# mobiusml/hqq

Hardware: NVIDIA H100
Metric: llama3_8b_4bit_gs64_decode_tokens_per_s (higher is better)
Workload: dtype f16

## Files before the change

hqq_b200/_lib.py:

```python
from __future__ import annotations

import ctypes
import os
from ctypes import c_char_p, c_float, c_int, c_int32, c_int64, c_size_t, c_void_p

import torch

_PKG_DIR = os.path.dirname(os.path.abspath(__file__))
LIB_PATH = os.path.join(_PKG_DIR, "libhqq_b200.so")

HQQ_F32, HQQ_F16, HQQ_BF16, HQQ_U8, HQQ_I32, HQQ_I64 = range(6)
HQQ_OK, HQQ_E_INVALID, HQQ_E_UNSUPPORTED, HQQ_E_WORKSPACE, HQQ_E_CUDA = 0, -1, -2, -3, -4

DTYPE_CODE = {
    torch.float32: HQQ_F32, torch.float16: HQQ_F16, torch.bfloat16: HQQ_BF16,
    torch.uint8: HQQ_U8, torch.int32: HQQ_I32, torch.int64: HQQ_I64,
}

SIGNATURES = {
    "hqq_b200_abi_version": (c_int, []),
    "hqq_b200_last_error": (c_char_p, []),
    "hqq_b200_pack": (c_int, [c_int, c_void_p, c_int, c_void_p, c_int64, c_int64, c_void_p]),
    "hqq_b200_unpack": (c_int, [c_int, c_void_p, c_void_p, c_int, c_int64, c_int64, c_void_p]),
    "hqq_b200_dequantize": (c_int, [c_void_p, c_void_p, c_void_p, c_void_p, c_int64, c_int64, c_int, c_int, c_int, c_int, c_void_p]),
    "hqq_b200_quantize_workspace_bytes": (c_size_t, [c_int64, c_int64, c_int, c_int, c_int, c_int]),
    "hqq_b200_quantize_shard_begin": (c_int, [c_void_p, c_int, c_int64, c_int64, c_int, c_int, c_int, c_int, c_float, c_float, c_int, c_void_p,
                                              c_void_p, c_size_t, c_void_p]),
    "hqq_b200_quantize_shard_finish": (c_int, [c_void_p, c_int, c_int64, c_int64, c_int, c_int, c_int, c_int, c_float, c_float, c_int, c_void_p,
                                               c_int64, c_void_p, c_void_p, c_void_p, c_void_p, c_void_p, c_void_p, c_size_t, c_void_p]),
    "hqq_b200_quantize": (c_int, [c_void_p, c_int, c_int64, c_int64, c_int, c_int, c_int, c_int, c_int, c_float, c_float, c_int,
                                  c_void_p, c_void_p, c_void_p, c_void_p, c_void_p, c_void_p, c_size_t, c_void_p]),
    "hqq_b200_quantize_ex": (c_int, [c_void_p, c_int, c_int64, c_int64, c_int, c_int, c_int, c_int, c_int, c_int, c_float, c_float,
                                     c_int, c_void_p, c_void_p, c_void_p, c_void_p, c_void_p, c_void_p, c_void_p, c_void_p,
                                     c_size_t, c_void_p]),
    "hqq_b200_linear_fwd_workspace_bytes": (c_size_t, [c_int64, c_int64, c_int64, c_int, c_int, c_int, c_int]),
    "hqq_b200_dense_gemm": (c_int, [c_void_p, c_void_p, c_void_p, c_void_p, c_int64, c_int64, c_int64, c_int, c_void_p]),
    "hqq_b200_lm_logprob_workspace_bytes": (c_size_t, [c_int64, c_int64]),
    "hqq_b200_lm_logprob": (c_int, [c_void_p, c_void_p, c_void_p, c_void_p, c_void_p, c_void_p, c_int64, c_int64, c_int64, c_int64, c_int, c_void_p]),
    "hqq_b200_linear_fwd": (c_int, [c_void_p, c_void_p, c_void_p, c_void_p, c_void_p, c_void_p, c_int64, c_int64, c_int64,
                                    c_int, c_int, c_int, c_int, c_void_p, c_size_t, c_void_p]),
    "hqq_b200_linear_fwd_multi": (c_int, [c_void_p, c_int, c_void_p, c_void_p, c_void_p, c_void_p, c_void_p, c_void_p, c_int64, c_int64,
                                          c_int, c_int, c_int, c_int, c_void_p, c_size_t, c_void_p]),
    "hqq_b200_linear_fwd_route": (c_int, [c_int64, c_int64, c_int64, c_int, c_int, c_int, c_int]),
    "hqq_b200_decode_linear_fwd": (c_int, [c_void_p, c_int, c_void_p, c_void_p, c_void_p, c_float, c_int, c_void_p, c_void_p, c_void_p, c_void_p,
                                           c_void_p, c_void_p, c_int64, c_int, c_int, c_int, c_void_p]),
    "hqq_b200_decode_linear_fwd_desc": (c_int, [c_void_p, c_void_p]),
    "hqq_b200_glue_add_rmsnorm_tp": (c_int, [c_void_p, c_void_p, c_void_p, c_int, c_int, c_int, c_void_p, c_void_p, c_int, c_float, c_int, c_void_p]),
    "hqq_b200_glue_add_rmsnorm": (c_int, [c_void_p, c_void_p, c_void_p, c_void_p, c_int, c_float, c_int, c_void_p]),
    "hqq_b200_glue_add_rmsnorm_rows": (c_int, [c_void_p, c_void_p, c_void_p, c_void_p, c_int, c_int, c_float, c_int, c_void_p]),
    "hqq_b200_glue_silu_mul": (c_int, [c_void_p, c_void_p, c_void_p, c_int, c_int, c_void_p]),
    "hqq_b200_glue_rope_attn_decode_batch": (c_int, [c_void_p, c_void_p, c_void_p, c_void_p, c_void_p, c_void_p, c_void_p, c_void_p, c_void_p,
                                                     c_int, c_int, c_int, c_int, c_int, c_int, c_void_p]),
    "hqq_b200_glue_rope_attn_decode": (c_int, [c_void_p, c_void_p, c_void_p, c_void_p, c_void_p, c_void_p, c_void_p, c_void_p, c_void_p,
                                               c_int, c_int, c_int, c_int, c_int, c_void_p]),
    "hqq_b200_glue_rope_attn_decode_split": (c_int, [c_void_p, c_void_p, c_void_p, c_void_p, c_void_p, c_void_p, c_void_p, c_void_p, c_void_p,
                                                     c_void_p, c_int, c_int, c_int, c_int, c_int, c_int, c_void_p]),
    "hqq_b200_glue_rope_attn_decode_split_workspace_bytes": (c_size_t, [c_int, c_int, c_int, c_int]),
    "hqq_b200_glue_rope_append_rows": (c_int, [c_void_p, c_void_p, c_void_p, c_void_p, c_void_p, c_void_p, c_void_p, c_void_p, c_int, c_int, c_int,
                                               c_int, c_int, c_int, c_int, c_int, c_void_p]),
    "hqq_b200_glue_rope_attn_decode_split_kv8": (c_int, [c_void_p] * 14 + [c_int] * 7 + [c_void_p]),
    "hqq_b200_glue_rope_append_rows_kv8": (c_int, [c_void_p] * 14 + [c_int] * 9 + [c_void_p]),
    "hqq_b200_glue_attn_prefill": (c_int, [c_void_p, c_void_p, c_void_p, c_void_p, c_int, c_int, c_int, c_int, c_int, c_int, c_int, c_int, c_void_p]),
    "hqq_b200_glue_rope_attn_decode_batch_seqpos": (c_int, [c_void_p] * 9 + [c_int] * 6 + [c_void_p]),
    "hqq_b200_glue_rope_attn_decode_split_seqpos": (c_int, [c_void_p] * 10 + [c_int] * 6 + [c_void_p]),
    "hqq_b200_glue_rope_attn_decode_split_kv8_seqpos": (c_int, [c_void_p] * 14 + [c_int] * 7 + [c_void_p]),
    "hqq_b200_glue_rope_append_rows_varlen": (c_int, [c_void_p] * 10 + [c_int] * 6 + [c_void_p]),
    "hqq_b200_glue_rope_append_rows_kv8_varlen": (c_int, [c_void_p] * 16 + [c_int] * 7 + [c_void_p]),
    "hqq_b200_glue_attn_prefill_varlen": (c_int, [c_void_p] * 6 + [c_int] * 6 + [c_void_p]),
    "hqq_b200_glue_rope_attn_decode_batch_paged": (c_int, [c_void_p] * 10 + [c_int] * 7 + [c_void_p]),
    "hqq_b200_glue_rope_attn_decode_split_paged": (c_int, [c_void_p] * 11 + [c_int] * 7 + [c_void_p]),
    "hqq_b200_glue_rope_attn_decode_split_kv8_paged": (c_int, [c_void_p] * 15 + [c_int] * 8 + [c_void_p]),
    "hqq_b200_glue_rope_append_rows_paged": (c_int, [c_void_p] * 11 + [c_int] * 7 + [c_void_p]),
    "hqq_b200_glue_rope_append_rows_kv8_paged": (c_int, [c_void_p] * 17 + [c_int] * 8 + [c_void_p]),
    "hqq_b200_glue_kv8_stage_paged": (c_int, [c_void_p] * 11 + [c_int] * 7 + [c_void_p]),
    "hqq_b200_glue_attn_prefill_paged": (c_int, [c_void_p] * 7 + [c_int] * 7 + [c_void_p]),
    "hqq_b200_glue_rope_append_rows_devpos": (c_int, [c_void_p] * 9 + [c_int] * 7 + [c_void_p]),
    "hqq_b200_glue_rope_append_rows_devpos_paged": (c_int, [c_void_p] * 10 + [c_int] * 8 + [c_void_p]),
    "hqq_b200_glue_attn_verify_split_workspace_bytes": (c_size_t, [c_int] * 5),
    "hqq_b200_glue_rope_append_rows_kv8_devpos": (c_int, [c_void_p] * 13 + [c_int] * 8 + [c_void_p]),
# ... 95 lines not shown
```

hqq_b200/csrc/linear.cu:

```cuda
#include "linear_internal.cuh"

namespace hqq {
bool small_route_ok(int64_t M, int64_t N, int64_t K, int gs, int nbits, int axis, int dtype);
size_t small_workspace_bytes(int64_t M);
int linear_small_multi(const void* x, int nprob, const void* const* Wq, const void* const* scale, const void* const* zero,
                       const void* const* bias, void* const* y, const int64_t* N, int64_t M, int64_t K, int gs, int nbits, int dtype,
                       void* ws, size_t ws_bytes, cudaStream_t st, int xop = 0, const void* x2 = nullptr, const void* xw = nullptr,
                       void* h_out = nullptr, float eps = 0.0f, const TpExchange* tpx = nullptr);
bool small_xop_ok(int64_t M, int64_t K);
bool gemm_route_ok(int64_t M, int64_t N, int64_t K, int gs, int nbits, int axis, int dtype);
size_t gemm_workspace_bytes(int64_t M, int64_t N, int64_t K, int gs, int nbits, int dtype);
int linear_gemm(const void* x, const void* Wq, const void* scale, const void* zero, const void* bias, void* y, int64_t M,
                int64_t N, int64_t K, int gs, int nbits, int dtype, void* ws, size_t ws_bytes, cudaStream_t st);
bool dense_route_ok(int64_t M, int64_t N, int64_t K, int dtype);
int linear_dense(const void* x, const void* W, const void* bias, void* y, int64_t M, int64_t N, int64_t K, int dtype, cudaStream_t st);
size_t lm_logprob_ws_bytes(int64_t M, int64_t N);
int lm_logprob(const void* x, const void* W, const int64_t* targets, float* lse, float* tgt, void* ws, int64_t M, int64_t N, int64_t K,
               int64_t index_offset, int dtype, cudaStream_t st);
}

using namespace hqq;

static bool dequant_ok(int64_t N, int64_t K, int gs, int nbits, int axis) {
  if (!valid_nbits(nbits) || !(axis == 0 || axis == 1) || gs <= 0 || N <= 0 || K <= 0 || (N * K) % gs != 0) return false;
  const int64_t R = axis == 1 ? N * K / gs : gs;
  return nbits == 3 || R % fields_of(nbits) == 0;
}

static size_t dense_ws_bytes(int64_t N, int64_t K, int dtype) { return (size_t)((N * K * (int64_t)dtype_size(dtype) + 255) & ~(int64_t)255); }

static bool prefer_small(int64_t M, int64_t N, int64_t K) {
  HQQ_ENV_KNOB(m, ([] { const char* e = getenv("HQQ_B200_SMALL_M_MAX"); return e ? atoi(e) : 0; })());
  if (m > 0) return M <= m;
  return M <= 16 || N * K <= (int64_t(1) << 24);
}

extern "C" int hqq_b200_linear_fwd_route(int64_t M, int64_t N, int64_t K, int group_size, int nbits, int axis, int dtype) {
  const bool small = small_route_ok(M, N, K, group_size, nbits, axis, dtype);
  if (small && (prefer_small(M, N, K) || !gemm_route_ok(M, N, K, group_size, nbits, axis, dtype))) return 1;
  if (gemm_route_ok(M, N, K, group_size, nbits, axis, dtype)) return 2;
  if (dequant_ok(N, K, group_size, nbits, axis) && dense_route_ok(M, N, K, dtype)) return 3;
  return 0;
// ... 58 lines not shown
  int rc = check_common(x, M, K, group_size, nbits, axis);
  if (rc) return rc;
  HQQ_REQUIRE(count >= 1 && count <= 4 && W_q && scale && zero && y && N, HQQ_E_INVALID, "hqq_b200_linear_fwd_multi: 1..4 matrices, non-null arrays");
  for (int i = 0; i < count; ++i) {
    if (!small_route_ok(M, N[i], K, group_size, nbits, axis, dtype)) {
      set_error("hqq_b200_linear_fwd_multi: matrix %d (N=%lld K=%lld gs=%d nbits=%d axis=%d dtype=%d M=%lld) is outside the fused small-M kernel",
                i, (long long)N[i], (long long)K, group_size, nbits, axis, dtype, (long long)M);
      return HQQ_E_UNSUPPORTED;
    }
  }
  return linear_small_multi(x, count, W_q, scale, zero, bias, y, N, M, K, group_size, nbits, dtype, workspace, workspace_bytes, (cudaStream_t)stream);
}

extern "C" int hqq_b200_decode_linear_fwd(const void* x, int x_op, const void* x2, const void* x_weight, void* h_out, float eps, int count,
                                          const void* const* W_q, const void* const* scale, const void* const* zero,
                                          const void* const* bias, void* const* y, const int64_t* N, int64_t K, int group_size, int nbits,
                                          int dtype, void* stream) {
  int rc = check_common(x, 1, K, group_size, nbits, 1);
  if (rc) return rc;
  HQQ_REQUIRE(count >= 1 && count <= 4 && W_q && scale && zero && y && N, HQQ_E_INVALID, "hqq_b200_decode_linear_fwd: 1..4 matrices, non-null arrays");
  HQQ_REQUIRE(x_op >= 0 && (x_op & 15) <= 2 && (x_op >> 4) <= 1, HQQ_E_INVALID,
              "hqq_b200_decode_linear_fwd: x_op must be 0 (none), 1 (add+rmsnorm) or 2 (silu*mul), optionally | HQQ_YOP_SILU_MUL_PAIR");
  for (int i = 0; i < count; ++i) {
    if (!small_route_ok(1, N[i], K, group_size, nbits, 1, dtype) || (x_op != 0 && !small_xop_ok(1, K))) {
      set_error("hqq_b200_decode_linear_fwd: matrix %d (N=%lld K=%lld gs=%d nbits=%d dtype=%d) is outside the fused M=1 kernel", i, (long long)N[i],
                (long long)K, group_size, nbits, dtype);
      return HQQ_E_UNSUPPORTED;
    }
  }
  return linear_small_multi(x, count, W_q, scale, zero, bias, y, N, 1, K, group_size, nbits, dtype, nullptr, 0, (cudaStream_t)stream, x_op, x2,
                            x_weight, h_out, eps);
}

extern "C" int hqq_b200_decode_linear_fwd_desc(const hqq_b200_decode_desc* d, void* stream) {
  HQQ_REQUIRE(d != nullptr, HQQ_E_INVALID, "hqq_b200_decode_linear_fwd_desc: null descriptor");
  int rc = check_common(d->x ? d->x : d->x_tagged, 1, d->K, d->group_size, d->nbits, 1);
  if (rc) return rc;
  HQQ_REQUIRE(d->count >= 1 && d->count <= 4 && d->W_q && d->scale && d->zero && d->y && d->N, HQQ_E_INVALID,
              "hqq_b200_decode_linear_fwd_desc: 1..4 matrices, non-null arrays");
  HQQ_REQUIRE(d->x_op >= 0 && (d->x_op & 15) <= 2 && (d->x_op >> 4) <= 1, HQQ_E_INVALID,
              "hqq_b200_decode_linear_fwd_desc: x_op must be 0, 1 or 2, optionally | HQQ_YOP_SILU_MUL_PAIR");
  HQQ_REQUIRE(d->x || ((d->x_op & 15) == 2 && d->x_tagged), HQQ_E_INVALID, "hqq_b200_decode_linear_fwd_desc: no activation given");
  for (int i = 0; i < d->count; ++i) {
    if (!small_route_ok(1, d->N[i], d->K, d->group_size, d->nbits, 1, d->dtype) || !small_xop_ok(1, d->K)) {
      set_error("hqq_b200_decode_linear_fwd_desc: matrix %d (N=%lld K=%lld gs=%d nbits=%d dtype=%d) is outside the fused M=1 kernel", i,
                (long long)d->N[i], (long long)d->K, d->group_size, d->nbits, d->dtype);
      return HQQ_E_UNSUPPORTED;
    }
  }
  TpExchange t{d->tp, d->rank, d->peer_data, d->red_data, d->y_tagged, d->x_tagged, d->x2_tagged, d->step_ctr, d->x_index, d->x_per_step};
  const bool exchange = d->step_ctr != nullptr;
  const void* x = d->x ? d->x : d->x_tagged;
  return linear_small_multi(x, d->count, d->W_q, d->scale, d->zero, d->bias, d->y, d->N, 1, d->K, d->group_size, d->nbits, d->dtype, nullptr, 0,
                            (cudaStream_t)stream, d->x_op, d->x2, d->x_weight, d->h_out, d->eps, exchange ? &t : nullptr);
}
```

hqq_b200/csrc/linear_small.cu:

```cuda
#include <string.h>
#include <type_traits>

#include "linear_internal.cuh"

namespace hqq {


constexpr int kMaxProb = 4;

struct SKProb {
  const uint8_t* Wq;
  const void* scale;
  const void* zero;
  const void* bias;
  void* y;
  uint32_t* ytag;
  int N;
  int step;
  int tile0;
};

struct SKArgs {
  SKProb p[kMaxProb];
  int nprob;
// ... 407 lines not shown
#pragma unroll
      for (int mt = 0; mt < MT; ++mt) {
        float4 acc = make_float4(0.f, 0.f, 0.f, 0.f);
#pragma unroll
        for (int w = 0; w < 8; ++w) {
          const float4 v = *reinterpret_cast<const float4*>(buf + (w * MT + mt) * 128 + lane * 4);
          acc.x += v.x; acc.y += v.y; acc.z += v.z; acc.w += v.w;
        }
        const int m0 = mt * 8 + 2 * c;
        if (m0 < a.M) {
          if (ok_a) MM::st(t.y, (long long)m0 * t.N + n_a, acc.x, t.bias, n_a);
          if (ok_b) MM::st(t.y, (long long)m0 * t.N + n_b, acc.z, t.bias, n_b);
        }
        if (m0 + 1 < a.M) {
          if (ok_a) MM::st(t.y, (long long)(m0 + 1) * t.N + n_a, acc.y, t.bias, n_a);
          if (ok_b) MM::st(t.y, (long long)(m0 + 1) * t.N + n_b, acc.w, t.bias, n_b);
        }
      }
    }
  }
  cp_async_wait<0>();
}

template <typename T, int NBITS, int GS, int ST, int MR = 0>
struct D1Cfg {
  static constexpr int F = 8 / NBITS, P = 16 / F, MPG = GS / 16, GPB = 256 / GS;
  static constexpr int NWV = (F == 1) ? 8 : 4;
  static constexpr int W_BYTES = ST * NWV * 256 * 16;
  static constexpr int M_BYTES = (MR & 1) ? ST * 8 * 4 * 8 * 16 : 0;
  static constexpr int P_BYTES = 2 * 8 * 16 * 4;
  static int smem(int K) { return W_BYTES + M_BYTES + P_BYTES + K * 2 + (K / GS) * 4; }
};

template <typename T, int NBITS, int GS, int ST, int MC, int MR = 0>
__global__ void __launch_bounds__(256, MC) linear_decode1_kernel(const __grid_constant__ SKArgs a) {
  using C = D1Cfg<T, NBITS, GS, ST, MR>;
  constexpr int F = C::F, P = C::P, MPG = C::MPG, GPB = C::GPB, NWV = C::NWV;
  using MM = MT16<T>;
  extern __shared__ __align__(16) uint8_t smem[];
  uint4* wring = reinterpret_cast<uint4*>(smem);
  uint4* mring = reinterpret_cast<uint4*>(smem + C::W_BYTES);
  float* part_s = reinterpret_cast<float*>(smem + C::W_BYTES + C::M_BYTES);
  T* xs = reinterpret_cast<T*>(smem + C::W_BYTES + C::M_BYTES + C::P_BYTES);
  float* xsum = reinterpret_cast<float*>(smem + C::W_BYTES + C::M_BYTES + C::P_BYTES + a.K * 2);

  const int tid = threadIdx.x, warp = tid >> 5, lane = tid & 31;
  const int r = lane >> 2, c = lane & 3;
  const int p = (F == 1) ? r : (r % P);
  const int fa = (F == 1) ? 0 : (r / P), fb = (F == 1) ? 0 : (F / 2 + r / P);
  Lanes<T, NBITS> lanes;
  lanes.init(8 - NBITS * (fa + 1), 8 - NBITS * (fb + 1));

  const int kb0 = a.KB * warp / 8, kb1 = a.KB * (warp + 1) / 8;
  const int upt = kb1 - kb0;
  const int n_tiles = (a.total_tiles - (int)blockIdx.x + (int)gridDim.x - 1) / (int)gridDim.x;
  if (n_tiles <= 0) return;

  struct Tile { const uint8_t* Wq; const T* scale; const T* zero; const T* bias; T* y; uint32_t* ytag; int N, step, tile0; };
  auto pick = [&](int pi, Tile& t) {
    const uint8_t* Wq = a.p[0].Wq; const void* sc = a.p[0].scale; const void* ze = a.p[0].zero; const void* bi = a.p[0].bias;
    void* y = a.p[0].y; uint32_t* yt = a.p[0].ytag; int N = a.p[0].N, step = a.p[0].step, tile0 = a.p[0].tile0;
#pragma unroll
    for (int i = 1; i < kMaxProb; ++i)
      if (pi == i) { Wq = a.p[i].Wq; sc = a.p[i].scale; ze = a.p[i].zero; bi = a.p[i].bias; y = a.p[i].y; yt = a.p[i].ytag; N = a.p[i].N; step = a.p[i].step; tile0 = a.p[i].tile0; }
    t.Wq = Wq; t.scale = reinterpret_cast<const T*>(sc); t.zero = reinterpret_cast<const T*>(ze);
    t.bias = reinterpret_cast<const T*>(bi); t.y = reinterpret_cast<T*>(y); t.ytag = yt; t.N = N; t.step = step; t.tile0 = tile0;
  };
  auto locate = [&](int gt, Tile& t) {
// ... 51 lines not shown
      --m_left;
      if (++m_k == upt) {
        m_k = 0; ++m_tile;
        if (m_left > 0) meta_setup();
      } else {
        ms_a += GPB; mz_a += GPB; ms_b += GPB; mz_b += GPB;
      }
    }
  };
  meta_fetch();
  auto issue = [&](int stage) {
    if (to_issue > 0) {
#pragma unroll
      for (int i = 0; i < 4; ++i) cp_async16(&wring[(stage * NWV + i) * 256 + tid], iw_a + i * 64);
      if (F == 1) {
#pragma unroll
        for (int i = 0; i < 4; ++i) cp_async16(&wring[(stage * NWV + 4 + i) * 256 + tid], iw_b + i * 64);
      }
      if constexpr ((MR & 1) != 0)
        cp_async16(&mring[((stage * 8 + warp) * 4 + c) * 8 + r], reinterpret_cast<const void*>(reinterpret_cast<uintptr_t>(im) & ~uintptr_t(15)));
      --to_issue;
      if (++i_k == upt) {
        i_k = 0; ++i_tile;
        if (to_issue > 0) issue_setup();
      } else {
        iw_a += 256; iw_b += 256;
        if constexpr ((MR & 1) != 0) im += GPB;
      }
    }
    cp_async_commit();
  };
#pragma unroll
  for (int s = 0; s < ST - 1; ++s) issue(s);
  pdl_launch_dependents();
  pdl_wait();
  uint32_t send_tag = 0, send_par = 0;
  if (a.step_ctr) {
    const uint32_t ex = (uint32_t)(*reinterpret_cast<volatile const int*>(a.step_ctr)) * (uint32_t)a.x_per_step + (uint32_t)a.x_index;
    send_tag = ex & 0xFFFFu;
    send_par = ex & 1u;
  }

  {
    const T* x = reinterpret_cast<const T*>(a.x);
    const T* x2 = reinterpret_cast<const T*>(a.x2);
    const int k_lo = kb0 * 256, k_hi = kb1 * 256;
    float inv = 1.0f;
    const uint32_t* red = nullptr;
    const uint32_t rtag = send_tag;
    if (a.xop == 1 && a.red_data) red = a.red_data + (size_t)send_par * a.tp * a.K;
    auto poll8 = [&](const uint32_t* src, Vec<T, 8>& out) {
      uint4 w0, w1;
      bool ok;
      do {
#ifdef HQQ_EMU
        memcpy(&w0, src, 16); memcpy(&w1, src + 4, 16);
#else
        asm volatile("ld.relaxed.sys.global.v4.u32 {%0,%1,%2,%3}, [%4];" : "=r"(w0.x), "=r"(w0.y), "=r"(w0.z), "=r"(w0.w) : "l"(src) : "memory");
        asm volatile("ld.relaxed.sys.global.v4.u32 {%0,%1,%2,%3}, [%4];" : "=r"(w1.x), "=r"(w1.y), "=r"(w1.z), "=r"(w1.w) : "l"(src + 4) : "memory");
#endif
        ok = ((w0.x >> 16) == rtag) & ((w0.y >> 16) == rtag) & ((w0.z >> 16) == rtag) & ((w0.w >> 16) == rtag) &
             ((w1.x >> 16) == rtag) & ((w1.y >> 16) == rtag) & ((w1.z >> 16) == rtag) & ((w1.w >> 16) == rtag);
      } while (!ok);
      const uint32_t ws[8] = {w0.x, w0.y, w0.z, w0.w, w1.x, w1.y, w1.z, w1.w};
#pragma unroll
      for (int j = 0; j < 8; ++j) {
        const unsigned short hb = (unsigned short)(ws[j] & 0xFFFFu);
        out.v[j] = *reinterpret_cast<const T*>(&hb);
      }
    };
    auto delta8 = [&](int k8, Vec<T, 8>& d) -> bool {
      if (red) {
        float acc[8];
#pragma unroll
        for (int j = 0; j < 8; ++j) acc[j] = 0.0f;
        for (int rr = 0; rr < a.tp; ++rr) {
          Vec<T, 8> p8;
          poll8(red + (size_t)rr * a.K + k8, p8);
#pragma unroll
          for (int j = 0; j < 8; ++j) acc[j] += to_f32<T>(p8.v[j]);
        }
#pragma unroll
        for (int j = 0; j < 8; ++j) d.v[j] = from_f32_t<T>(acc[j]);
        return true;
      }
      if (x2) { d = *reinterpret_cast<const Vec<T, 8>*>(x2 + k8); return true; }
      return false;
    };
    auto put_permuted = [&](int k8, const Vec<T, 8>& v) {
      Vec<T, 8> w;
      w.v[0] = v.v[0]; w.v[1] = v.v[2]; w.v[2] = v.v[1]; w.v[3] = v.v[3];
      w.v[4] = v.v[4]; w.v[5] = v.v[6]; w.v[6] = v.v[5]; w.v[7] = v.v[7];
      *reinterpret_cast<Vec<T, 8>*>(xs + k8) = w;
    };
    if (a.xop == 1) {
      const T* xw = reinterpret_cast<const T*>(a.xw);
      T* hout = reinterpret_cast<T*>(a.h_out);
      const int kg0 = k_lo + lane * 8;
      Vec<T, 8> g0, g1;
      if (kg0 < k_hi) g0 = *reinterpret_cast<const Vec<T, 8>*>(xw + kg0);
      if (kg0 + 256 < k_hi) g1 = *reinterpret_cast<const Vec<T, 8>*>(xw + kg0 + 256);
      float ss = 0.0f;
      for (int ka = tid * 8; ka < a.K; ka += 2 * 256 * 8) {
        const int kb = ka + 256 * 8;
        const bool has_b = kb < a.K;
        Vec<T, 8> va = *reinterpret_cast<const Vec<T, 8>*>(x + ka), vb, da, db;
        if (has_b) vb = *reinterpret_cast<const Vec<T, 8>*>(x + kb);
        const bool add_a = delta8(ka, da);
        const bool add_b = has_b && delta8(kb, db);
        if (add_a) {
#pragma unroll
          for (int j = 0; j < 8; ++j) va.v[j] = from_f32_t<T>(to_f32<T>(va.v[j]) + to_f32<T>(da.v[j]));
        }
        if (add_b) {
#pragma unroll
          for (int j = 0; j < 8; ++j) vb.v[j] = from_f32_t<T>(to_f32<T>(vb.v[j]) + to_f32<T>(db.v[j]));
        }
        *reinterpret_cast<Vec<T, 8>*>(xs + ka) = va;
        if (has_b) *reinterpret_cast<Vec<T, 8>*>(xs + kb) = vb;
        if (hout && blockIdx.x == 0) {
          *reinterpret_cast<Vec<T, 8>*>(hout + ka) = va;
          if (has_b) *reinterpret_cast<Vec<T, 8>*>(hout + kb) = vb;
        }
#pragma unroll
        for (int j = 0; j < 8; ++j) { const float f = to_f32<T>(va.v[j]); ss += f * f; }
        if (has_b) {
#pragma unroll
          for (int j = 0; j < 8; ++j) { const float f = to_f32<T>(vb.v[j]); ss += f * f; }
        }
      }
#pragma unroll
      for (int o = 16; o > 0; o >>= 1) ss += __shfl_xor_sync(0xffffffffu, ss, o);
      if (lane == 0) part_s[warp] = ss;
      __syncthreads();
// ... 128 lines not shown
          const uint32_t word = (send_tag << 16) | (uint32_t)(*reinterpret_cast<const unsigned short*>(&pv));
          if (a.peer_data[0]) {
            const size_t off = ((size_t)send_par * a.tp + a.rank) * t.N + n;
#pragma unroll
            for (int dst = 0; dst < 8; ++dst)
              if (dst < a.tp) HQQ_ST_RELAXED_SYS(a.peer_data[dst] + off, word);
          }
          if (t.ytag) HQQ_ST_RELAXED_SYS(t.ytag + (size_t)send_par * t.N + n, word);
        }
      }
    }
  }
  cp_async_wait<0>();
}

template <typename T, int NBITS, int GS, int MT>
static int launch_sk(SKArgs& a, cudaStream_t st) {
  using C = SKCfg<T, NBITS, GS, MT>;
  int rc = reserve_smem<linear_small_kernel<T, NBITS, GS, MT>>(C::SMEM);
  if (rc) return rc;
  static int per_sm[kMaxDevices] = {};
  int& occ = per_sm[current_device()];
  if (!occ) {
    int n = 0;
    cudaError_t e = cudaOccupancyMaxActiveBlocksPerMultiprocessor(&n, linear_small_kernel<T, NBITS, GS, MT>, 256, C::SMEM);
    HQQ_REQUIRE(e == cudaSuccess && n > 0, HQQ_E_CUDA, "hqq_b200_linear_fwd: occupancy query failed: %s", cudaGetErrorString(e));
    occ = n > 2 ? 2 : n;
  }
  const int max_grid = sm_count() * occ;
  return launch_pdl("hqq_b200_linear_fwd/small", linear_small_kernel<T, NBITS, GS, MT>, dim3((unsigned)(a.total_tiles < max_grid ? a.total_tiles : max_grid)),
                    dim3(256), C::SMEM, st, a);
}

template <typename T, int NBITS, int GS, int ST, int MC, int MR = 0>
static int launch_d1(SKArgs& a, cudaStream_t st) {
  const int smem = D1Cfg<T, NBITS, GS, ST, MR>::smem(a.K);
  int rc = reserve_smem<linear_decode1_kernel<T, NBITS, GS, ST, MC, MR>>(smem);
  if (rc) return rc;
  int per_sm = MC;
  while (per_sm > 1 && (smem + 1024) * per_sm > 227 * 1024) --per_sm;
  const int max_grid = sm_count() * per_sm;
  return launch_pdl("hqq_b200_linear_fwd/decode1", linear_decode1_kernel<T, NBITS, GS, ST, MC, MR>,
                    dim3((unsigned)(a.total_tiles < max_grid ? a.total_tiles : max_grid)), dim3(256), smem, st, a);
}

bool small_xop_ok(int64_t M, int64_t K) { return M == 1 && K <= 16384; }

template <typename T, int NBITS, int GS>
static int sk_mt(SKArgs& a, cudaStream_t st) {
  if (small_xop_ok(a.M, a.K)) {
    if constexpr (NBITS == 8) {
      return launch_d1<T, NBITS, GS, 2, 2>(a, st);
    } else {
      if constexpr (GS == 64) {
        if (a.K % 512 == 0) {
          bool ok = true;
          for (int i = 0; i < a.nprob; ++i) ok = ok && aligned(a.p[i].scale, 16) && aligned(a.p[i].zero, 16);
          if (ok) return launch_d1<T, NBITS, GS, 4, 2, 1>(a, st);
        }
      }
      return launch_d1<T, NBITS, GS, 4, 2>(a, st);
    }
  }
  if (a.M <= 8) return launch_sk<T, NBITS, GS, 1>(a, st);
  if (a.M <= 16) return launch_sk<T, NBITS, GS, 2>(a, st);
  return launch_sk<T, NBITS, GS, 4>(a, st);
}

template <typename T, int NBITS>
static int sk_gs(SKArgs& a, int gs, cudaStream_t st) {
  switch (gs) {
    case 64: return sk_mt<T, NBITS, 64>(a, st);
    case 128: return sk_mt<T, NBITS, 128>(a, st);
  }
  return HQQ_E_UNSUPPORTED;
}

template <typename T>
static int sk_bits(SKArgs& a, int gs, int nbits, cudaStream_t st) {
  switch (nbits) {
    case 8:
      if constexpr (std::is_same<T, __half>::value) return sk_gs<T, 8>(a, gs, st);
      else return HQQ_E_UNSUPPORTED;
    case 4: return sk_gs<T, 4>(a, gs, st);
    case 2: return sk_gs<T, 2>(a, gs, st);
    case 1: return sk_gs<T, 1>(a, gs, st);
  }
  return HQQ_E_UNSUPPORTED;
}

bool small_route_ok(int64_t M, int64_t N, int64_t K, int gs, int nbits, int axis, int dtype) {
  if (axis != 1) return false;
  if (dtype != HQQ_F16 && dtype != HQQ_BF16) return false;
  if (!(nbits == 8 || nbits == 4 || nbits == 2 || nbits == 1)) return false;
  if (nbits == 8 && dtype == HQQ_BF16) return false;
  if (!(gs == 64 || gs == 128)) return false;
  if (M < 1 || M > 32) return false;
  if (K % 256 != 0 || K % gs != 0) return false;
  if (N % (8 / nbits) != 0) return false;
  if (N > (1 << 28) || K > (1 << 28)) return false;
  return true;
}

size_t small_workspace_bytes(int64_t) { return 0; }

int linear_small_multi(const void* x, int nprob, const void* const* Wq, const void* const* scale, const void* const* zero,
                       const void* const* bias, void* const* y, const int64_t* N, int64_t M, int64_t K, int gs, int nbits, int dtype,
                       void* ws, size_t ws_bytes, cudaStream_t st, int xop, const void* x2, const void* xw, void* h_out, float eps,
                       const TpExchange* tpx) {
  HQQ_REQUIRE(nprob >= 1 && nprob <= kMaxProb, HQQ_E_INVALID, "hqq_b200_linear_fwd_multi: 1..%d matrices per launch (got %d)", kMaxProb, nprob);
  HQQ_REQUIRE(aligned(x, 16), HQQ_E_INVALID, "hqq_b200_linear_fwd: x must be 16-byte aligned");
  (void)ws; (void)ws_bytes;
  const int F = 8 / nbits, P = 16 / F;
  SKArgs a;
  a.nprob = nprob; a.x = x; a.M = (int)M; a.K = (int)K; a.Gk = (int)(K / gs); a.KB = (int)(K / 256);
  const int yop = xop >> 4;
  xop &= 15;
  a.xop = xop; a.yop = yop; a.x2 = x2; a.xw = xw; a.h_out = h_out; a.eps = eps;
  if (yop) {
    HQQ_REQUIRE(yop == 1, HQQ_E_INVALID, "hqq_b200_decode_linear_fwd: unknown epilogue %d", yop);
    HQQ_REQUIRE(nprob == 2 && N[0] == N[1], HQQ_E_INVALID, "hqq_b200_decode_linear_fwd: the silu*mul epilogue pairs exactly two matrices of equal N");
    if (!(small_xop_ok(M, K) && nbits < 8) || (tpx && (tpx->peer_data || tpx->y_tagged))) {
      set_error("hqq_b200_decode_linear_fwd: the silu*mul epilogue needs the M == 1 kernel, nbits < 8 and plain outputs");
      return HQQ_E_UNSUPPORTED;
    }
  }
  a.tp = 1; a.rank = 0; a.red_data = nullptr; a.xtag = nullptr; a.x2tag = nullptr; a.step_ctr = nullptr; a.x_index = 0; a.x_per_step = 1;
  for (int i = 0; i < 8; ++i) a.peer_data[i] = nullptr;
  if (tpx && !tpx->step_ctr) tpx = nullptr;
  if (tpx) {
    HQQ_REQUIRE(small_xop_ok(M, K) && nprob >= 1, HQQ_E_UNSUPPORTED, "hqq_b200_decode_linear_fwd_desc: needs the M == 1 kernel");
    HQQ_REQUIRE(tpx->tp >= 1 && tpx->tp <= 8 && tpx->rank >= 0 && tpx->rank < tpx->tp && tpx->step_ctr && tpx->x_per_step > 0, HQQ_E_INVALID,
                "hqq_b200_decode_linear_fwd_desc: bad tp/rank/step counter");
    a.tp = tpx->tp; a.rank = tpx->rank; a.step_ctr = tpx->step_ctr; a.x_index = tpx->x_index; a.x_per_step = tpx->x_per_step;
    if (tpx->peer_data) {
      HQQ_REQUIRE(nprob == 1, HQQ_E_INVALID, "hqq_b200_decode_linear_fwd_desc: the scatter side takes exactly one matrix");
      for (int i = 0; i < tpx->tp; ++i) a.peer_data[i] = reinterpret_cast<uint32_t*>(tpx->peer_data[i]);
// ... 27 lines not shown
```

include/hqq_b200.h:

```cpp
#ifndef HQQ_B200_H
#define HQQ_B200_H

#include <stddef.h>
#include <stdint.h>

#ifdef __cplusplus
extern "C" {
#endif

#define HQQ_B200_ABI_VERSION 2

enum {
  HQQ_F32 = 0,
  HQQ_F16 = 1,
  HQQ_BF16 = 2,
  HQQ_U8 = 3,
  HQQ_I32 = 4,
  HQQ_I64 = 5
};

enum {
  HQQ_OK = 0,
  HQQ_E_INVALID = -1,
  HQQ_E_UNSUPPORTED = -2,
// ... 49 lines not shown
int hqq_b200_dense_gemm(const void* x, const void* W, const void* bias, void* y, int64_t M, int64_t N, int64_t K,
                        int dtype, void* stream);

size_t hqq_b200_lm_logprob_workspace_bytes(int64_t M, int64_t N);
int hqq_b200_lm_logprob(const void* x, const void* W, const int64_t* targets, float* lse, float* tgt, void* workspace, int64_t M,
                        int64_t N, int64_t K, int64_t index_offset, int dtype, void* stream);

int hqq_b200_linear_fwd_multi(const void* x, int count, const void* const* W_q, const void* const* scale,
                              const void* const* zero, const void* const* bias, void* const* y, const int64_t* N,
                              int64_t M, int64_t K, int group_size, int nbits, int axis, int dtype,
                              void* workspace, size_t workspace_bytes, void* stream);

int hqq_b200_linear_fwd_route(int64_t M, int64_t N, int64_t K, int group_size, int nbits,
                              int axis, int dtype);

#define HQQ_YOP_SILU_MUL_PAIR 16
int hqq_b200_decode_linear_fwd(const void* x, int x_op, const void* x2, const void* x_weight, void* h_out, float eps,
                               int count, const void* const* W_q, const void* const* scale, const void* const* zero,
                               const void* const* bias, void* const* y, const int64_t* N, int64_t K,
                               int group_size, int nbits, int dtype, void* stream);
typedef struct hqq_b200_decode_desc {
  const void* x; int x_op; const void* x2; const void* x_weight; void* h_out; float eps;
  int count; const void* const* W_q; const void* const* scale; const void* const* zero; const void* const* bias;
  void* const* y; const int64_t* N; int64_t K; int group_size; int nbits; int dtype;
  int tp; int rank;
  void* const* peer_data;
  const void* red_data;
  void* const* y_tagged;
  const void* x_tagged;
  const void* x2_tagged;
  const int* step_ctr; int x_index; int x_per_step;
} hqq_b200_decode_desc;
int hqq_b200_decode_linear_fwd_desc(const hqq_b200_decode_desc* desc, void* stream);
int hqq_b200_glue_add_rmsnorm_tp(void* h, const void* red_data, int* step_ctr, int x_index, int x_per_step, int tp,
                                 const void* weight, void* y, int H, float eps, int dtype, void* stream);
int hqq_b200_glue_add_rmsnorm(void* h, const void* delta, const void* weight, void* y,
                              int H, float eps, int dtype, void* stream);
int hqq_b200_glue_add_rmsnorm_rows(void* h, const void* delta, const void* weight, void* y,
                                   int rows, int H, float eps, int dtype, void* stream);
int hqq_b200_glue_silu_mul(const void* gate, const void* up, void* y, int n, int dtype, void* stream);
int hqq_b200_glue_rope_attn_decode(const void* q, const void* k, const void* v,
                                   const void* cos_table, const void* sin_table,
                                   void* k_cache, void* v_cache, const int64_t* pos, void* out,
                                   int n_q_heads, int n_kv_heads, int cache_len, int head_dim,
                                   int dtype, void* stream);
int hqq_b200_glue_rope_attn_decode_batch(const void* q, const void* k, const void* v,
                                         const void* cos_table, const void* sin_table,
                                         void* k_cache, void* v_cache, const int64_t* pos, void* out,
                                         int n_q_heads, int n_kv_heads, int cache_len, int head_dim,
                                         int batch, int dtype, void* stream);
int hqq_b200_glue_rope_attn_decode_split(const void* q, const void* k, const void* v,
                                         const void* cos_table, const void* sin_table,
                                         void* k_cache, void* v_cache, const int64_t* pos, void* out, void* workspace,
                                         int n_q_heads, int n_kv_heads, int cache_len, int head_dim,
                                         int batch, int dtype, void* stream);
size_t hqq_b200_glue_rope_attn_decode_split_workspace_bytes(int n_q_heads, int n_kv_heads, int head_dim, int batch);
int hqq_b200_glue_rope_attn_decode_split_kv8(const void* q, const void* k, const void* v,
                                             const void* cos_table, const void* sin_table,
                                             void* k_q, void* k_scale, void* k_zero, void* v_q, void* v_scale, void* v_zero,
                                             const int64_t* pos, void* out, void* workspace,
                                             int n_q_heads, int n_kv_heads, int cache_len, int head_dim, int group_size,
                                             int batch, int dtype, void* stream);
int hqq_b200_glue_rope_append_rows(const void* q, const void* k, const void* v,
                                   const void* cos_table, const void* sin_table,
                                   void* k_cache, void* v_cache, void* q_out, int pos0, int T,
                                   int n_q_heads, int n_kv_heads, int cache_len, int head_dim,
// ... 186 lines not shown
```

Measured before the change: 428.8.

## Rework decode1 kernel occupancy, add deeper pipeline stage, hoist norm-weight loads

Result: faster. 434.9, median of 6 (+1.4%).

```diff
diff --git a/hqq_b200/_lib.py b/hqq_b200/_lib.py
--- a/hqq_b200/_lib.py
+++ b/hqq_b200/_lib.py
@@ -45,6 +45,7 @@
     "hqq_b200_decode_linear_fwd": (c_int, [c_void_p, c_int, c_void_p, c_void_p, c_void_p, c_float, c_int, c_void_p, c_void_p, c_void_p, c_void_p,
                                            c_void_p, c_void_p, c_int64, c_int, c_int, c_int, c_void_p]),
     "hqq_b200_decode_linear_fwd_desc": (c_int, [c_void_p, c_void_p]),
+    "hqq_b200_decode_linear_footprint": (c_int, [c_int64, c_int, c_int, c_int, c_int, c_void_p]),
     "hqq_b200_glue_add_rmsnorm_tp": (c_int, [c_void_p, c_void_p, c_void_p, c_int, c_int, c_int, c_void_p, c_void_p, c_int, c_float, c_int, c_void_p]),
     "hqq_b200_glue_add_rmsnorm": (c_int, [c_void_p, c_void_p, c_void_p, c_void_p, c_int, c_float, c_int, c_void_p]),
     "hqq_b200_glue_add_rmsnorm_rows": (c_int, [c_void_p, c_void_p, c_void_p, c_void_p, c_int, c_int, c_float, c_int, c_void_p]),
diff --git a/hqq_b200/csrc/linear.cu b/hqq_b200/csrc/linear.cu
--- a/hqq_b200/csrc/linear.cu
+++ b/hqq_b200/csrc/linear.cu
@@ -8,6 +8,7 @@
                        void* ws, size_t ws_bytes, cudaStream_t st, int xop = 0, const void* x2 = nullptr, const void* xw = nullptr,
                        void* h_out = nullptr, float eps = 0.0f, const TpExchange* tpx = nullptr);
 bool small_xop_ok(int64_t M, int64_t K);
+int decode1_footprint(int64_t K, int gs, int nbits, int dtype, int occupancy_smem, int* out);
 bool gemm_route_ok(int64_t M, int64_t N, int64_t K, int gs, int nbits, int axis, int dtype);
 size_t gemm_workspace_bytes(int64_t M, int64_t N, int64_t K, int gs, int nbits, int dtype);
 int linear_gemm(const void* x, const void* Wq, const void* scale, const void* zero, const void* bias, void* y, int64_t M,
@@ -132,6 +133,10 @@
                             x_weight, h_out, eps);
 }
 
+extern "C" int hqq_b200_decode_linear_footprint(int64_t K, int group_size, int nbits, int dtype, int occupancy_smem, int* out) {
+  return decode1_footprint(K, group_size, nbits, dtype, occupancy_smem, out);
+}
+
 extern "C" int hqq_b200_decode_linear_fwd_desc(const hqq_b200_decode_desc* d, void* stream) {
   HQQ_REQUIRE(d != nullptr, HQQ_E_INVALID, "hqq_b200_decode_linear_fwd_desc: null descriptor");
   int rc = check_common(d->x ? d->x : d->x_tagged, 1, d->K, d->group_size, d->nbits, 1);
diff --git a/hqq_b200/csrc/linear_small.cu b/hqq_b200/csrc/linear_small.cu
--- a/hqq_b200/csrc/linear_small.cu
+++ b/hqq_b200/csrc/linear_small.cu
@@ -463,8 +463,12 @@
   static int smem(int K) { return W_BYTES + M_BYTES + P_BYTES + K * 2 + (K / GS) * 4; }
 };
 
-template <typename T, int NBITS, int GS, int ST, int MC, int MR = 0>
-__global__ void __launch_bounds__(256, MC) linear_decode1_kernel(const __grid_constant__ SKArgs a) {
+constexpr int kD1Threads = 256;
+constexpr int kD1SmemBudget = 227 * 1024 / 2 - 1024;
+constexpr int kD1RegBudget = 64 * 1024 / 2;
+
+template <typename T, int NBITS, int GS, int ST, int MR = 0>
+__global__ void __launch_bounds__(kD1Threads, 2) linear_decode1_kernel(const __grid_constant__ SKArgs a) {
   using C = D1Cfg<T, NBITS, GS, ST, MR>;
   constexpr int F = C::F, P = C::P, MPG = C::MPG, GPB = C::GPB, NWV = C::NWV;
   using MM = MT16<T>;
@@ -582,6 +586,14 @@
   };
 #pragma unroll
   for (int s = 0; s < ST - 1; ++s) issue(s);
+  const int k_lo = kb0 * 256, k_hi = kb1 * 256;
+  const int kg0 = k_lo + lane * 8;
+  Vec<T, 8> g0, g1;
+  if (a.xop == 1) {
+    const T* xw = reinterpret_cast<const T*>(a.xw);
+    if (kg0 < k_hi) g0 = *reinterpret_cast<const Vec<T, 8>*>(xw + kg0);
+    if (kg0 + 256 < k_hi) g1 = *reinterpret_cast<const Vec<T, 8>*>(xw + kg0 + 256);
+  }
   pdl_launch_dependents();
   pdl_wait();
   uint32_t send_tag = 0, send_par = 0;
@@ -594,7 +606,6 @@
   {
     const T* x = reinterpret_cast<const T*>(a.x);
     const T* x2 = reinterpret_cast<const T*>(a.x2);
-    const int k_lo = kb0 * 256, k_hi = kb1 * 256;
     float inv = 1.0f;
     const uint32_t* red = nullptr;
     const uint32_t rtag = send_tag;
@@ -646,10 +657,6 @@
     if (a.xop == 1) {
       const T* xw = reinterpret_cast<const T*>(a.xw);
       T* hout = reinterpret_cast<T*>(a.h_out);
-      const int kg0 = k_lo + lane * 8;
-      Vec<T, 8> g0, g1;
-      if (kg0 < k_hi) g0 = *reinterpret_cast<const Vec<T, 8>*>(xw + kg0);
-      if (kg0 + 256 < k_hi) g1 = *reinterpret_cast<const Vec<T, 8>*>(xw + kg0 + 256);
       float ss = 0.0f;
       for (int ka = tid * 8; ka < a.K; ka += 2 * 256 * 8) {
         const int kb = ka + 256 * 8;
@@ -844,16 +851,72 @@
                     dim3(256), C::SMEM, st, a);
 }
 
-template <typename T, int NBITS, int GS, int ST, int MC, int MR = 0>
+template <typename T, int NBITS, int GS, int ST, int MR>
+struct D1 {
+  using Cfg = D1Cfg<T, NBITS, GS, ST, MR>;
+  static constexpr auto kernel = linear_decode1_kernel<T, NBITS, GS, ST, MR>;
+};
+
+template <typename T, int NBITS, int GS, typename Fn>
+static int d1_select(int K, bool meta16, Fn&& fn) {
+  if constexpr (NBITS == 8) {
+    return fn(D1<T, NBITS, GS, 2, 0>{});
+  } else {
+    if constexpr (GS == 64) {
+      if (K % 512 == 0 && meta16) {
+        if (D1Cfg<T, NBITS, GS, 5, 1>::smem(K) <= kD1SmemBudget) return fn(D1<T, NBITS, GS, 5, 1>{});
+        if (D1Cfg<T, NBITS, GS, 4, 1>::smem(K) <= kD1SmemBudget) return fn(D1<T, NBITS, GS, 4, 1>{});
+      }
+    }
+    return fn(D1<T, NBITS, GS, 4, 0>{});
+  }
+}
+
+static int d1_ctas_per_sm() {
+  HQQ_ENV_KNOB(n, ([] { const char* e = getenv("HQQ_B200_D1_CTAS_PER_SM"); return e ? atoi(e) : 0; })());
+  return n == 2 ? 2 : 1;
+}
+
+template <typename D>
+static int d1_attrs(int& regs, int& static_smem) {
+  static int r_[kMaxDevices] = {}, s_[kMaxDevices] = {};
+  const int dev = current_device();
+  if (!r_[dev]) {
+#ifdef HQQ_EMU
+    r_[dev] = 128; s_[dev] = 0;
+#else
+    cudaFuncAttributes fa;
+    cudaError_t e = cudaFuncGetAttributes(&fa, D::kernel);
+    HQQ_REQUIRE(e == cudaSuccess, HQQ_E_CUDA, "hqq_b200_linear_fwd/decode1: cudaFuncGetAttributes failed: %s", cudaGetErrorString(e));
+    HQQ_REQUIRE(fa.numRegs * kD1Threads <= kD1RegBudget && fa.maxThreadsPerBlock >= kD1Threads, HQQ_E_CUDA,
+                "hqq_b200_linear_fwd/decode1: %d registers x %d threads exceed half of the SM's register file", fa.numRegs, kD1Threads);
+    r_[dev] = fa.numRegs; s_[dev] = (int)fa.sharedSizeBytes;
+#endif
+  }
+  regs = r_[dev];
+  static_smem = s_[dev];
+  return HQQ_OK;
+}
+
+template <typename D>
+static int d1_footprint(int K, int& regs, int& smem) {
+  int static_smem = 0;
+  int rc = d1_attrs<D>(regs, static_smem);
+  if (rc) return rc;
+  const int dyn = D::Cfg::smem(K);
+  smem = static_smem + dyn;
+  HQQ_REQUIRE(smem <= kD1SmemBudget, HQQ_E_CUDA, "hqq_b200_linear_fwd/decode1: %d bytes of shared memory at K = %d exceed half of the SM's", smem, K);
+  return reserve_smem<D::kernel>(dyn);
+}
+
+template <typename D>
 static int launch_d1(SKArgs& a, cudaStream_t st) {
-  const int smem = D1Cfg<T, NBITS, GS, ST, MR>::smem(a.K);
-  int rc = reserve_smem<linear_decode1_kernel<T, NBITS, GS, ST, MC, MR>>(smem);
+  int regs = 0, smem = 0;
+  int rc = d1_footprint<D>(a.K, regs, smem);
   if (rc) return rc;
-  int per_sm = MC;
-  while (per_sm > 1 && (smem + 1024) * per_sm > 227 * 1024) --per_sm;
-  const int max_grid = sm_count() * per_sm;
-  return launch_pdl("hqq_b200_linear_fwd/decode1", linear_decode1_kernel<T, NBITS, GS, ST, MC, MR>,
-                    dim3((unsigned)(a.total_tiles < max_grid ? a.total_tiles : max_grid)), dim3(256), smem, st, a);
+  const int max_grid = sm_count() * d1_ctas_per_sm();
+  return launch_pdl("hqq_b200_linear_fwd/decode1", D::kernel, dim3((unsigned)(a.total_tiles < max_grid ? a.total_tiles : max_grid)),
+                    dim3(kD1Threads), D::Cfg::smem(a.K), st, a);
 }
 
 bool small_xop_ok(int64_t M, int64_t K) { return M == 1 && K <= 16384; }
@@ -861,18 +924,9 @@
 template <typename T, int NBITS, int GS>
 static int sk_mt(SKArgs& a, cudaStream_t st) {
   if (small_xop_ok(a.M, a.K)) {
-    if constexpr (NBITS == 8) {
-      return launch_d1<T, NBITS, GS, 2, 2>(a, st);
-    } else {
-      if constexpr (GS == 64) {
-        if (a.K % 512 == 0) {
-          bool ok = true;
-          for (int i = 0; i < a.nprob; ++i) ok = ok && aligned(a.p[i].scale, 16) && aligned(a.p[i].zero, 16);
-          if (ok) return launch_d1<T, NBITS, GS, 4, 2, 1>(a, st);
-        }
-      }
-      return launch_d1<T, NBITS, GS, 4, 2>(a, st);
-    }
+    bool meta16 = true;
+    for (int i = 0; i < a.nprob; ++i) meta16 = meta16 && aligned(a.p[i].scale, 16) && aligned(a.p[i].zero, 16);
+    return d1_select<T, NBITS, GS>(a.K, meta16, [&](auto d) -> int { return launch_d1<decltype(d)>(a, st); });
   }
   if (a.M <= 8) return launch_sk<T, NBITS, GS, 1>(a, st);
   if (a.M <= 16) return launch_sk<T, NBITS, GS, 2>(a, st);
@@ -915,6 +969,58 @@
 }
 
 size_t small_workspace_bytes(int64_t) { return 0; }
+
+template <typename T, int NBITS, int GS>
+static int d1_query(int K, int occupancy_smem, int* out) {
+  return d1_select<T, NBITS, GS>(K, true, [&](auto d) -> int {
+    using D = decltype(d);
+    int regs = 0, smem = 0;
+    int rc = d1_footprint<D>(K, regs, smem);
+    if (rc) return rc;
+    const int dyn = occupancy_smem > D::Cfg::smem(K) ? occupancy_smem : D::Cfg::smem(K);
+    rc = reserve_smem<D::kernel>(dyn);
+    if (rc) return rc;
+    int n = 0;
+    cudaError_t e = cudaOccupancyMaxActiveBlocksPerMultiprocessor(&n, D::kernel, kD1Threads, dyn);
+    HQQ_REQUIRE(e == cudaSuccess, HQQ_E_CUDA, "hqq_b200_decode_linear_footprint: occupancy query failed: %s", cudaGetErrorString(e));
+    out[0] = regs; out[1] = kD1Threads; out[2] = smem; out[3] = d1_ctas_per_sm(); out[4] = n;
+    out[5] = D::Cfg::W_BYTES / (D::Cfg::NWV * 256 * 16); out[6] = D::Cfg::M_BYTES ? 1 : 0;
+    return HQQ_OK;
+  });
+}
+
+template <typename T, int NBITS>
+static int d1_query_gs(int K, int gs, int occupancy_smem, int* out) {
+  switch (gs) {
+    case 64: return d1_query<T, NBITS, 64>(K, occupancy_smem, out);
+    case 128: return d1_query<T, NBITS, 128>(K, occupancy_smem, out);
+  }
+  return HQQ_E_UNSUPPORTED;
+}
+
+int decode1_footprint(int64_t K, int gs, int nbits, int dtype, int occupancy_smem, int* out) {
+  HQQ_REQUIRE(out, HQQ_E_INVALID, "hqq_b200_decode_linear_footprint: null output");
+  if (!small_route_ok(1, 8, K, gs, nbits, 1, dtype) || !small_xop_ok(1, K)) {
+    set_error("hqq_b200_decode_linear_footprint: K=%lld gs=%d nbits=%d dtype=%d is outside the fused M=1 kernel", (long long)K, gs, nbits, dtype);
+    return HQQ_E_UNSUPPORTED;
+  }
+  const int k = (int)K;
+  if (dtype == HQQ_F16) {
+    switch (nbits) {
+      case 8: return d1_query_gs<__half, 8>(k, gs, occupancy_smem, out);
+      case 4: return d1_query_gs<__half, 4>(k, gs, occupancy_smem, out);
+      case 2: return d1_query_gs<__half, 2>(k, gs, occupancy_smem, out);
+      case 1: return d1_query_gs<__half, 1>(k, gs, occupancy_smem, out);
+    }
+  } else {
+    switch (nbits) {
+      case 4: return d1_query_gs<__nv_bfloat16, 4>(k, gs, occupancy_smem, out);
+      case 2: return d1_query_gs<__nv_bfloat16, 2>(k, gs, occupancy_smem, out);
+      case 1: return d1_query_gs<__nv_bfloat16, 1>(k, gs, occupancy_smem, out);
+    }
+  }
+  return HQQ_E_UNSUPPORTED;
+}
 
 int linear_small_multi(const void* x, int nprob, const void* const* Wq, const void* const* scale, const void* const* zero,
                        const void* const* bias, void* const* y, const int64_t* N, int64_t M, int64_t K, int gs, int nbits, int dtype,
diff --git a/include/hqq_b200.h b/include/hqq_b200.h
--- a/include/hqq_b200.h
+++ b/include/hqq_b200.h
@@ -105,6 +105,8 @@
   const int* step_ctr; int x_index; int x_per_step;
 } hqq_b200_decode_desc;
 int hqq_b200_decode_linear_fwd_desc(const hqq_b200_decode_desc* desc, void* stream);
+
+int hqq_b200_decode_linear_footprint(int64_t K, int group_size, int nbits, int dtype, int occupancy_smem, int* out);
 int hqq_b200_glue_add_rmsnorm_tp(void* h, const void* red_data, int* step_ctr, int x_index, int x_per_step, int tp,
                                  const void* weight, void* y, int H, float eps, int dtype, void* stream);
 int hqq_b200_glue_add_rmsnorm(void* h, const void* delta, const void* weight, void* y,
```
